# david-wb/tiny-diffusion

Measured on AMD Instinct MI355X. Metric: train images/s (q_sample+fwd+MSE+bwd+allreduce+Adam), MNIST 28x28 UNet fp32; 1000-step sample latency in `sample`, higher is better.
Workload: dtype f32; 1 GPU; diffusion.py unconditional MNIST 28x28 UNet, fp32, train step, batch 256/GPU (BASELINE.json configs[1]); global_batch=256, per_gpu_batch=256, parallelism=dp1

## Files before the change

include/tdx.h:

```cpp
#ifndef TDX_H
#define TDX_H

#include <stddef.h>
#include <stdint.h>

#ifdef __cplusplus
extern "C" {
#endif

#define TDX_VERSION 400

#define TDX_E_BADARG (-1)
#define TDX_E_SHAPE (-2)
#define TDX_E_WORKSPACE (-3)
#define TDX_E_STATE (-4)

typedef void* tdx_stream_t;

int tdx_version(void);
const char* tdx_error_string(int code);


int tdx_q_sample(const float* x0, const float* noise, const int64_t* t,
                 const float* sqrt_ac, const float* sqrt_1mac, float* x_t,
// ... 70 lines not shown
int tdx_initial_conv_input_grad(const float* g_out, const float* w, float* g_x, int B, int H, int W, int cin,
                                int cout, tdx_stream_t stream);
int tdx_final_conv_forward(const float* in, const float* w, const float* bias, float* out, int B, int H, int W,
                           int cout, tdx_stream_t stream);
int tdx_final_conv_backward(const float* in, const float* g_out, const float* w, float* g_in, float* dw, float* db,
                            float* scratch, int B, int H, int W, int cout, tdx_stream_t stream);

int tdx_conv3x3_fwd(const float* in, const float* wpk, const float* bias, float* out,
                    int B, int H, int W, int cin, int cout, int flags,
                    const float* in_scale, const float* in_shift,
                    const float* out_scale, const float* out_shift,
                    float* stats_partial, tdx_stream_t stream);
int tdx_conv3x3_fwd_splitk(const float* in, const float* wpk, const float* bias, float* out,
                           int B, int H, int W, int cin, int cout, int flags,
                           const float* in_scale, const float* in_shift,
                           const float* out_scale, const float* out_shift,
                           float* scratch, size_t scratch_floats, tdx_stream_t stream);
size_t tdx_conv3x3_splitk_scratch_floats(int B, int H, int W, int cin, int cout);
int tdx_conv3x3_wino_ok(int B, int H, int W, int cin, int cout);
int tdx_pack_conv3x3_wino(const float* w_oihw, float* u_fwd, float* u_dgrad, int cout, int cin, tdx_stream_t stream);
int tdx_conv3x3_fwd_wino(const float* in, const float* u, const float* bias, float* out, int B, int H, int W,
                         int cin, int cout, int flags, const float* out_scale, const float* out_shift,
                         float* stats_partial, tdx_stream_t stream);
int tdx_conv3x3_fwd_wino_infer(const float* in, const float* u, const float* bias, float* out, int B, int H, int W,
                               int cin, int cout, const float* out_scale, const float* out_shift, float* scratch,
                               size_t scratch_floats, tdx_stream_t stream);
int tdx_conv3x3_train_algo(int B, int H, int W, int cin, int cout, int role);
int tdx_conv3x3_infer_algo(int B, int H, int W, int cin, int cout);
int tdx_conv3x3_wgrad_wino_splits(int B, int H, int W, int cin, int cout);
int tdx_conv3x3_wgrad_wino(const float* in, const float* dy, float* dw_slabs, int B, int H, int W, int cin, int cout,
                           tdx_stream_t stream);
int tdx_conv3x3_wino_stat_tiles(int B, int H, int W);
int tdx_conv3x3_wino_stat_tile_rows(int B, int H, int W);
int tdx_pack_conv3x3_tiled(const float* w_oihw, float* w_tiled, int cout, int cin, tdx_stream_t stream);
int tdx_conv3x3_fwd_infer(const float* in, const float* w_tiled, const float* bias, float* out, int B, int H, int W,
                          int cin, int cout, const float* out_scale, const float* out_shift, float* scratch,
                          size_t scratch_floats, tdx_stream_t stream);
size_t tdx_conv3x3_infer_scratch_floats(int B, int H, int W, int cin, int cout);
int tdx_conv3x3_fwd_train(const float* in, const float* wpk, const float* bias, float* out, int B, int H, int W,
                          int cin, int cout, int flags, float* stats_partial, float* scratch,
                          size_t scratch_floats, tdx_stream_t stream);
size_t tdx_conv3x3_train_scratch_floats(int B, int H, int W, int cin, int cout);
int tdx_conv3x3_stat_tiles(int B, int H, int W, int cin, int cout);
int tdx_conv3x3_stat_tile_rows(int B, int H, int W, int cin, int cout);
int tdx_conv3x3_shape_ok(int B, int H, int W, int cin, int cout);
int tdx_conv3x3_tile_shape(int B, int H, int W, int cin, int cout, int role);
// ... 193 lines not shown
```

tiny_diffusion_amd/_lib.py:

```python
from __future__ import annotations

import ctypes as C
import os

import torch

from . import _build

_c_float_p = C.c_void_p
_c_i64_p = C.c_void_p
_ptr = C.c_void_p


class TdxError(RuntimeError):
    pass


def _load():
    path = _build.LIB
    if not os.path.exists(path):
        if os.environ.get("TDX_NO_AUTOBUILD"):
            raise TdxError(
                f"{path} not found: build it with `python -m tiny_diffusion_amd._build` "
                "(there is no CPU fallback for the HIP path)"
# ... 26 lines not shown
    "tdx_p_sample_step": (C.c_int, [_ptr, _ptr, _ptr, _ptr, _ptr, _ptr, C.c_int64, _ptr]),
    "tdx_p_sample_step_philox": (C.c_int, [_ptr, _ptr, _ptr, _ptr, _ptr, C.c_int64, C.c_uint64, _ptr]),
    "tdx_u8_gather_normalize": (C.c_int, [_ptr, _ptr, _ptr, C.c_int, C.c_int, C.c_float, C.c_float, _ptr]),
    "tdx_mse_loss": (C.c_int, [_ptr, _ptr, _ptr, _ptr, C.c_float, C.c_int64, _ptr]),
    "tdx_mse_scratch_bytes": (C.c_size_t, []),
    "tdx_mse_loss_grad": (C.c_int, [_ptr, _ptr, _ptr, _ptr, C.c_float, C.c_int64, _ptr, _ptr]),
    "tdx_adam_step": (C.c_int, [_ptr, _ptr, _ptr, _ptr, C.c_int64, C.c_float, C.c_float, C.c_float,
                                C.c_float, C.c_int, C.c_float, _ptr]),
    "tdx_adam_clip_scratch_bytes": (C.c_size_t, []),
    "tdx_adam_step_clip": (C.c_int, [_ptr, _ptr, _ptr, _ptr, C.c_int64, C.c_float, C.c_float, C.c_float, C.c_float,
                                     C.c_int, C.c_float, C.c_float, _ptr, _ptr, _ptr]),
    "tdx_edge_conv_wgrad_scratch_floats": (C.c_size_t, [C.c_int] * 3),
    "tdx_initial_conv_forward": (C.c_int, [_ptr, _ptr, _ptr, _ptr, C.c_int, C.c_int, C.c_int, C.c_int, C.c_int, _ptr]),
    "tdx_initial_conv_backward": (C.c_int, [_ptr, _ptr, _ptr, _ptr, _ptr, C.c_int, C.c_int, C.c_int, C.c_int, C.c_int,
                                            _ptr]),
    "tdx_final_conv_forward": (C.c_int, [_ptr, _ptr, _ptr, _ptr, C.c_int, C.c_int, C.c_int, C.c_int, _ptr]),
    "tdx_final_conv_backward": (C.c_int, [_ptr, _ptr, _ptr, _ptr, _ptr, _ptr, _ptr, C.c_int, C.c_int, C.c_int, C.c_int,
                                          _ptr]),
    "tdx_pack_conv3x3": (C.c_int, [_ptr, _ptr, _ptr, C.c_int, C.c_int, _ptr]),
    "tdx_conv3x3_wino_ok": (C.c_int, [C.c_int] * 5),
    "tdx_pack_conv3x3_wino": (C.c_int, [_ptr, _ptr, _ptr, C.c_int, C.c_int, _ptr]),
    "tdx_conv3x3_fwd_wino": (C.c_int, [_ptr, _ptr, _ptr, _ptr, C.c_int, C.c_int, C.c_int, C.c_int, C.c_int, C.c_int, _ptr,
                                       _ptr, _ptr, _ptr]),
    "tdx_conv3x3_fwd_wino_infer": (C.c_int, [_ptr, _ptr, _ptr, _ptr, C.c_int, C.c_int, C.c_int, C.c_int, C.c_int, _ptr, _ptr,
                                             _ptr, C.c_size_t, _ptr]),
    "tdx_conv3x3_train_algo": (C.c_int, [C.c_int] * 6),
    "tdx_conv3x3_infer_algo": (C.c_int, [C.c_int] * 5),
    "tdx_conv3x3_wgrad_wino_splits": (C.c_int, [C.c_int] * 5),
    "tdx_conv3x3_wgrad_wino": (C.c_int, [_ptr, _ptr, _ptr, C.c_int, C.c_int, C.c_int, C.c_int, C.c_int, _ptr]),
    "tdx_conv3x3_wino_stat_tiles": (C.c_int, [C.c_int] * 3),
    "tdx_conv3x3_wino_stat_tile_rows": (C.c_int, [C.c_int] * 3),
    "tdx_pack_conv3x3_tiled": (C.c_int, [_ptr, _ptr, C.c_int, C.c_int, _ptr]),
    "tdx_conv3x3_fwd_infer": (C.c_int, [_ptr, _ptr, _ptr, _ptr, C.c_int, C.c_int, C.c_int, C.c_int, C.c_int, _ptr, _ptr,
                                        _ptr, C.c_size_t, _ptr]),
    "tdx_conv3x3_infer_scratch_floats": (C.c_size_t, [C.c_int] * 5),
    "tdx_conv3x3_fwd": (C.c_int, [_ptr, _ptr, _ptr, _ptr, C.c_int, C.c_int, C.c_int, C.c_int, C.c_int,
                                  C.c_int, _ptr, _ptr, _ptr, _ptr, _ptr, _ptr]),
    "tdx_conv3x3_fwd_splitk": (C.c_int, [_ptr, _ptr, _ptr, _ptr, C.c_int, C.c_int, C.c_int, C.c_int, C.c_int,
                                         C.c_int, _ptr, _ptr, _ptr, _ptr, _ptr, C.c_size_t, _ptr]),
    "tdx_conv3x3_splitk_scratch_floats": (C.c_size_t, [C.c_int] * 5),
    "tdx_conv3x3_fwd_train": (C.c_int, [_ptr, _ptr, _ptr, _ptr, C.c_int, C.c_int, C.c_int, C.c_int, C.c_int, C.c_int,
                                        _ptr, _ptr, C.c_size_t, _ptr]),
    "tdx_conv3x3_train_scratch_floats": (C.c_size_t, [C.c_int] * 5),
    "tdx_conv3x3_stat_tiles": (C.c_int, [C.c_int] * 5),
    "tdx_conv3x3_stat_tile_rows": (C.c_int, [C.c_int] * 5),
    "tdx_conv3x3_wgrad_splits": (C.c_int, [C.c_int] * 5),
# ... 142 lines not shown
```

tiny_diffusion_amd/csrc/conv3x3.hip:

```cpp
#include "internal.h"
#include <cstring>

#define BK 32
#define BKP 36

#include "conv_shared.h"

template <int BM, int BN, int EPI>
__global__ void __launch_bounds__(256)
conv3x3_igemm_kernel(ConvArgs a) {
  constexpr int WGM = 2, WGN = 2;
  constexpr int WTM = BM / WGM, WTN = BN / WGN;
  constexpr int TM = WTM / 32, TN = WTN / 32;
  constexpr int AI = BM / 32, BI = BN / 32;
  static_assert(TM >= 1 && TN >= 1, "wave tile must hold a 32x32 MFMA tile");

  extern __shared__ __attribute__((aligned(16))) float smem[];
  float* As = smem;
  float* Bs = smem + 2 * BM * BKP;

  const int tid = threadIdx.x;
  const int lane = tid & 63, wave = tid >> 6;
  const int l31 = lane & 31, half = lane >> 5;
  const int wm = wave / WGN, wn = wave % WGN;
// ... 737 lines not shown
  if (!strcmp(key, "time_proj_early")) { g_tdx_time_proj_early = value != 0; return 0; }
  if (!strcmp(key, "time_stage_diag")) { g_tdx_time_stage = value == 6 ? 6 : 14; return 0; }
  if (!strcmp(key, "time_l1_impl")) { g_tdx_time_l1_impl = value; return 0; }
  if (!strcmp(key, "input_copy")) { g_tdx_input_copy = value; return 0; }
  if (!strcmp(key, "conv_dbg")) { g_conv_dbg = value; return 0; }
  if (!strcmp(key, "bf16_materialize")) { g_tdx_bf16_materialize = value ? 1 : 0; return 0; }
  if (!strcmp(key, "bf16_thin")) { g_tdx_bf16_thin = value < 0 ? 0 : value; return 0; }
  if (!strcmp(key, "bf16_ring")) { g_tdx_bf16_ring = value ? 1 : 0; return 0; }
  if (!strcmp(key, "bf16_wgrad9")) { g_tdx_wgrad9 = value ? 1 : 0; return 0; }
  if (!strcmp(key, "bf16_wgrad_swz")) { g_tdx_wgrad_bf16s = value ? 1 : 0; return 0; }
  if (!strcmp(key, "conv_stamp")) { g_conv_stamp = value; g_tdx_probe_stamp = value; return 0; }
  if (!strcmp(key, "wgrad_small")) { g_wgrad_small = value; return 0; }
  if (!strcmp(key, "wino")) { g_tdx_wino = value != 0; return 0; }
  if (!strcmp(key, "wino_infer")) { g_tdx_wino_infer = value != 0; return 0; }
  if (!strcmp(key, "wino_infer_min_units")) { g_tdx_wino_infer_min_units = value >= 0 ? value : 700; return 0; }
  if (!strcmp(key, "wino_infer_ovh")) { g_wino_infer_ovh = value >= 0 ? value : 2; return 0; }
  if (!strcmp(key, "wino_infer_red")) { g_wino_infer_red = value >= 0 ? value : 3; return 0; }
  if (!strcmp(key, "wino_wgrad")) { g_tdx_wino_wgrad = value != 0; return 0; }
  if (!strcmp(key, "wino_wgrad_min_tiles")) { g_tdx_wino_wgrad_min_tiles = value > 0 ? value : 1024; return 0; }
  if (!strcmp(key, "wino_wgrad_target")) { g_tdx_wino_wgrad_target = value > 0 ? value : 512; return 0; }
  if (!strcmp(key, "wino_min_wgs")) { g_tdx_wino_min_wgs = value > 0 ? value : 1; return 0; }
  if (!strcmp(key, "wino_rows")) { g_tdx_wino_rows = value != 0; return 0; }
  if (!strcmp(key, "wino_rows_min_stages")) { g_tdx_wino_rows_min_stages = value > 0 ? value : 16; return 0; }
  if (!strcmp(key, "infer_ring")) { g_tdx_infer_ring = value != 0; return 0; }
  if (!strcmp(key, "infer_stages")) { g_infer_stages = value == 3 ? 3 : 4; return 0; }
  if (!strcmp(key, "infer_splits")) { g_infer_splits = value > 0 ? value : 0; return 0; }
  if (!strcmp(key, "infer_ovh")) { g_infer_ovh = value >= 0 ? value : 4; return 0; }
  if (!strcmp(key, "infer_red")) { g_infer_red = value >= 0 ? value : 12; return 0; }
  if (!strcmp(key, "infer_cus")) { g_tdx_infer_cus = value > 0 && value <= 256 ? value : 256; return 0; }
  if (!strcmp(key, "wgrad9_wgs")) { g_wgrad9_wgs = value > 0 ? value : 0; return 0; }
  if (!strcmp(key, "wgrad_target")) { g_wgrad_target = value > 0 ? value : 2048; return 0; }
  if (!strcmp(key, "wgrad_target_big")) { g_wgrad_target_big = value > 0 ? value : 0; return 0; }
  return TDX_E_BADARG;
}

static TileCfg pick_tile(int64_t M, int cout) {
  const TileCfg cands[3] = {{128, 128}, {128, 64}, {64, 64}};
  if (g_force_tile >= 1 && g_force_tile <= 3 && cout % cands[g_force_tile - 1].bn == 0)
    return cands[g_force_tile - 1];
  for (int i = 0; i < 3; ++i) {
    if (cout % cands[i].bn) continue;
    if (i == 2) return cands[i];
    const int64_t tiles = ((M + cands[i].bm - 1) / cands[i].bm) * (cout / cands[i].bn);
    if (tiles < g_min_tiles) continue;
    const int64_t rounds = (tiles + 255) / 256;
    if ((double)(rounds * 256) <= 1.035 * (double)tiles) return cands[i];
// ... 1165 lines not shown
```

tiny_diffusion_amd/csrc/conv3x3_wino.hip:

```cpp
#include "internal.h"
#include "conv_shared.h"

extern unsigned* g_tdx_diag_buffer;
extern size_t g_tdx_diag_bytes;
extern int g_tdx_probe_stamp;

constexpr int WT = 64;
constexpr int WN = 64;
constexpr int WK = 8;
constexpr int A_ST = 16 * WT * WK;
constexpr int B_ST = 16 * WN * WK;
constexpr int STAGE = A_ST + B_ST;

struct WinoArgs {
  const float* in;
  const float* u;
  const float* bias;
  float* out;
  const float* out_scale;
  const float* out_shift;
  float* stats;
  int B, H, W, Cin, Cout, th, tw, NT, tilesN, M;
  float rcp_tpi, rcp_tw;
  int per;
  int compact;
  unsigned long long* stamps;
};

constexpr int OLD = 68;
constexpr int TAB_OFF = 2 * STAGE;
typedef unsigned u32x4 __attribute__((ext_vector_type(4)));

template <int EPI, int XH = -1>
__device__ __forceinline__ void wino_epilogue(const WinoArgs& a, float* out, const float* bias, f32x16 (&acc)[16], float* smem,
                                              int tblk, int n0, int wm, int wn, int l31, int half, int tid,
                                              const f32x4* xin = nullptr) {
#if defined(__HIP_DEVICE_COMPILE__)
  const unsigned* tab = reinterpret_cast<const unsigned*>(smem + TAB_OFF);
  const int cl = wn * 32 + l31, col = n0 + cl;
  const float bv = bias ? bias[col] : 0.f;
  float osc = 1.f, osh = 0.f;
  if (EPI == EPI_BNRELU) { osc = a.out_scale[col]; osh = a.out_shift[col]; }
  float csum = 0.f, cnt = 0.f;
  float* ot = smem;
  f32x4 pv[8];
#pragma unroll
  for (int r = 0; r < 16; ++r) {
    if (XH >= 0 && (r & 3) == 0) {
#pragma unroll
      for (int p = 0; p < 8; ++p) pv[p] = xin[(p * 4 + (r >> 2)) * 64];
    }
    auto M = [&](int p) { return XH >= 0 && (p >> 3) != XH ? pv[p & 7][r & 3] : acc[p][r]; };
    float s0[4], s1[4];
#pragma unroll
    for (int nu = 0; nu < 4; ++nu) {
      s0[nu] = M(0 + nu) + M(4 + nu) + M(8 + nu);
// ... 9 lines not shown
      const bool ok = (m >> q) & 1u;
      if (XH < 0) ot[(tl * 4 + q) * OLD + cl] = val;
      csum += ok ? val : 0.f;
      cnt += ok ? 1.f : 0.f;
      y[q] = ok ? val : 0.f;
    }
    acc[0][r] = y[0]; acc[1][r] = y[1]; acc[4][r] = y[2]; acc[5][r] = y[3];
    acc[2][r] = (m & 1u) ? 1.f : 0.f;
    acc[3][r] = (m & 2u) ? 1.f : 0.f;
    acc[6][r] = (m & 4u) ? 1.f : 0.f;
    acc[7][r] = (m & 8u) ? 1.f : 0.f;
  }
  if (XH >= 0) {
    __syncthreads();
#pragma unroll
    for (int r = 0; r < 16; ++r) {
      const int tl = wm * 32 + (r & 3) + 8 * (r >> 2) + 4 * half;
      ot[(tl * 4 + 0) * OLD + cl] = acc[0][r]; ot[(tl * 4 + 1) * OLD + cl] = acc[1][r];
      ot[(tl * 4 + 2) * OLD + cl] = acc[4][r]; ot[(tl * 4 + 3) * OLD + cl] = acc[5][r];
    }
  }
  __syncthreads();
  {
    const auto rsrc_out = __builtin_amdgcn_make_buffer_rsrc(out, 0, (int)((int64_t)a.M * a.Cout * 4), 0x00020000);
    const int c4 = (tid & 15) * 4, q = (tid >> 4) & 3;
    const unsigned qoff = (unsigned)((((q >> 1) * a.W + (q & 1)) * a.Cout + n0 + c4) * 4);
    const uint2* tab2 = reinterpret_cast<const uint2*>(tab);
    const float* src = ot + (tid >> 4) * OLD + c4;
#pragma unroll
    for (int i = 0; i < 16; ++i) {
      const uint2 e = tab2[4 * i + (tid >> 6)];
      const unsigned off = ((e.y >> q) & 1u) ? e.x + qoff : 0x80000000u;
      const f32x4 v = *reinterpret_cast<const f32x4*>(src + i * 16 * OLD);
      __builtin_amdgcn_raw_buffer_store_b128(__builtin_bit_cast(u32x4, v), rsrc_out, off, 0, 0);
    }
  }
  if (EPI == EPI_STATS) {
    float* red = smem + 256 * OLD;
    const float s = csum + __shfl_xor(csum, 32, 64);
    const float n = cnt + __shfl_xor(cnt, 32, 64);
    if (half == 0) { red[wm * 64 + cl] = s; red[128 + wm * 64 + cl] = n; }
    __syncthreads();
    if (tid < 64) {
      const float ts = red[tid] + red[64 + tid];
      const float tn = red[128 + tid] + red[192 + tid];
      red[256 + tid] = tn > 0.f ? ts / tn : 0.f;
      a.stats[((size_t)tblk * 2 + 0) * a.Cout + n0 + tid] = ts;
    }
    __syncthreads();
    const float mean = red[256 + cl];
    float q = 0.f;
#pragma unroll
    for (int r = 0; r < 16; ++r) {
      const float d0 = acc[0][r] - mean, d1 = acc[1][r] - mean, d2 = acc[4][r] - mean, d3 = acc[5][r] - mean;
      q = fmaf(d0 * acc[2][r], d0, q); q = fmaf(d1 * acc[3][r], d1, q);
// ... 17 lines not shown

__device__ __forceinline__ int div_rcp(int n, int d, float r, int* rem) {
  int q = (int)((float)n * r);
  int m = n - q * d;
  if (m < 0) { --q; m += d; }
  else if (m >= d) { ++q; m -= d; }
  *rem = m;
  return q;
}

template <int EPI, bool SPLITK, bool ROWS>
__global__ void __launch_bounds__(256)
conv3x3_wino_kernel(WinoArgs a) {
#if defined(__HIP_DEVICE_COMPILE__)
  static_assert(!ROWS || (!SPLITK && EPI != EPI_BNRELU), "the row split serves the training launches only");
  typedef __attribute__((address_space(3))) void* lds_ptr_t;
  extern __shared__ __attribute__((aligned(16))) float smem[];
  const unsigned long long t_entry = a.stamps ? __builtin_amdgcn_s_memrealtime() : 0ull;
  const int tid = threadIdx.x;
  const int lane = tid & 63;
  const int wave = __builtin_amdgcn_readfirstlane(tid >> 6);
  const int l31 = lane & 31, half = lane >> 5;
  const int wm = ROWS ? wave & 1 : wave >> 1, wn = ROWS ? wave >> 1 : wave & 1;
  const int xb = blockIdx.x / (8 * a.tilesN), xr = blockIdx.x % (8 * a.tilesN);
  const int tblk = a.compact ? (int)blockIdx.x / a.tilesN : xb * 8 + (xr & 7);
  const int nblk = a.compact ? (int)blockIdx.x - tblk * a.tilesN : xr >> 3;
  const int T0 = tblk * WT;
  if (T0 >= a.NT) return;
  const int n0 = nblk * WN;
  const int tpi = a.th * a.tw;

  if (tid < WT) {
    const int T = T0 + tid;
    const bool tv = T < a.NT;
    int rem, tx;
    const int b = div_rcp(T, tpi, a.rcp_tpi, &rem);
    const int ty = div_rcp(rem, a.tw, a.rcp_tw, &tx);
    const bool r1 = 2 * ty + 1 < a.H, c1 = 2 * tx + 1 < a.W;
    unsigned* tab = reinterpret_cast<unsigned*>(smem + TAB_OFF);
    tab[2 * tid] = tv ? (unsigned)(((b * a.H + 2 * ty) * a.W + 2 * tx) * a.Cout * 4) : 0u;
    tab[2 * tid + 1] = tv ? (1u | (c1 ? 2u : 0u) | (r1 ? 4u : 0u) | (r1 && c1 ? 8u : 0u)) : 0u;
  }

  const auto rsrc_in = __builtin_amdgcn_make_buffer_rsrc(const_cast<float*>(a.in), 0, (int)((int64_t)a.M * a.Cin * 4), 0x00020000);
  const auto rsrc_u = __builtin_amdgcn_make_buffer_rsrc(const_cast<float*>(a.u), 0, a.Cout * 16 * a.Cin * 4, 0x00020000);
  constexpr unsigned OOB = 0x80000000u;
  unsigned a_off[4][2];
#pragma unroll
  for (int g = 0; g < 2; ++g) {
// ... 222 lines not shown
          if (p < 12) { xop(2 * p); xop(2 * p + 1); }
          else piece(2 * (p - 12), cb, s + 2);
          __builtin_amdgcn_sched_barrier(0);
          acc[p] = __builtin_amdgcn_mfma_f32_32x32x2f32(v[p][2], bq[cur][2], acc[p], 0, 0, 0);
          if (p < 12) bq[(p + 2) % 5] = *reinterpret_cast<const f32x4*>(Bb + (p + 2) * 512);
          if (p == 12) { nbq[0] = *reinterpret_cast<const f32x4*>(Bn); nbq[1] = *reinterpret_cast<const f32x4*>(Bn + 512); }
          if (p == 13) {
#pragma unroll
            for (int c = 0; c < 4; ++c) d[12 + c] = *reinterpret_cast<const f32x4*>(An + (12 + c) * 512);
          }
          if (p == 14) { v[0] = sub4(t1[0], t1[2]); v[1] = add4(t1[1], t1[2]); }
          if (p == 15) piece(7, cb, s + 2);
          __builtin_amdgcn_sched_barrier(0);
          acc[p] = __builtin_amdgcn_mfma_f32_32x32x2f32(v[p][3], bq[cur][3], acc[p], 0, 0, 0);
          if (p >= 12 && p < 15) piece(2 * (p - 12) + 1, cb, s + 2);
          __builtin_amdgcn_sched_barrier(0);
        }
      };
      if (PEEL) stage(std::true_type{}, 0);
      for (int s = PEEL ? 1 : 0; s < ns; ++s) stage(std::false_type{}, s);
      asm volatile("s_waitcnt vmcnt(0) lgkmcnt(0)\n\ts_barrier" ::: "memory");
    }
    if (a.stamps) { t_loop = __builtin_amdgcn_s_memrealtime(); c_loop = __builtin_amdgcn_s_memtime() - c_loop; }
    if (SPLITK)
      wino_epilogue<EPI_PLAIN>(a, a.out + (size_t)blockIdx.y * (size_t)a.M * a.Cout, nullptr, acc, smem, tblk, n0, wm, wn, l31, half, tid);
    else
      wino_epilogue<EPI>(a, a.out, a.bias, acc, smem, tblk, n0, wm, wn, l31, half, tid);
  }
  if (a.stamps && tid == 0) {
    asm volatile("s_waitcnt vmcnt(0)" ::: "memory");
    unsigned long long* o = a.stamps + 8 * ((size_t)blockIdx.y * gridDim.x + blockIdx.x);
    o[0] = t_entry; o[1] = t_issued; o[2] = t_landed; o[3] = t_loop; o[4] = __builtin_amdgcn_s_memrealtime();
    o[5] = c_loop;
    o[6] = __builtin_amdgcn_s_getreg(4 | (0 << 6) | (31 << 11));
    o[7] = __builtin_amdgcn_s_getreg(20 | (0 << 6) | (3 << 11)) & 0xf;
  }
#endif
}

__global__ void __launch_bounds__(512) pack_wino_batch_kernel(TdxWinoPackBatch b) {
  int u = 0;
  while (u + 1 < b.count && (int)blockIdx.x >= b.start[u + 1]) ++u;
  const int cin = b.cin[u], cout = b.cout[u], cin_real = b.cin_real[u];
  const int blk = blockIdx.x - b.start[u];
  const int nkb = cin / 8;
  const int cb = blk / nkb, kb = blk - cb * nkb;
  const int cl = threadIdx.x >> 3, k8 = threadIdx.x & 7;
  const int co = cb * 64 + cl, ci = kb * 8 + k8;
  float g[9];
// ... 67 lines not shown
  TDX_CHECK_LAUNCH();
  return 0;
}

int tdx_pack_conv3x3_wino_pad(const float* w_oihw, float* u_fwd, float* u_dgrad, int cout, int cin_real, int cin,
                              tdx_stream_t stream) {
  if (!w_oihw || cout <= 0 || cin <= 0 || cin_real <= 0 || cin_real > cin) return TDX_E_BADARG;
  if (cin % 64 || cout % 64) return TDX_E_SHAPE;
  if (!u_fwd && !u_dgrad) return 0;
  TdxWinoPackBatch b{};
  b.count = 1;
  b.w[0] = w_oihw; b.uf[0] = u_fwd; b.ud[0] = u_dgrad; b.cout[0] = cout; b.cin[0] = cin; b.cin_real[0] = cin_real;
  return tdx_pack_conv3x3_wino_batch(&b, stream);
}

extern "C" int tdx_pack_conv3x3_wino(const float* w_oihw, float* u_fwd, float* u_dgrad, int cout, int cin,
                                     tdx_stream_t stream) {
  return tdx_pack_conv3x3_wino_pad(w_oihw, u_fwd, u_dgrad, cout, cin, cin, stream);
}

int g_tdx_wino_rows = 1;
int g_tdx_wino_rows_min_stages = 16;

int tdx_conv3x3_wino_launch(const float* in, const float* u, const float* bias, float* out, int B, int H, int W,
                            int cin, int cout, int flags, const float* out_scale, const float* out_shift,
                            float* stats_partial, int splits, int per, tdx_stream_t stream) {
  if (!in || !u || !out) return TDX_E_BADARG;
  if (!tdx_conv3x3_wino_ok(B, H, W, cin, cout)) return TDX_E_SHAPE;
  if (flags & ~(TDX_CONV_OUT_BNRELU | TDX_CONV_OUT_STATS)) return TDX_E_BADARG;
  if ((flags & TDX_CONV_OUT_BNRELU) && (!out_scale || !out_shift)) return TDX_E_BADARG;
  if ((flags & TDX_CONV_OUT_STATS) && (!stats_partial || (flags & TDX_CONV_OUT_BNRELU))) return TDX_E_BADARG;
  if (splits < 1 || (splits > 1 && (per < 1 || (int64_t)per * (splits - 1) >= cin / WK))) return TDX_E_BADARG;
  WinoArgs a{};
  a.in = in; a.u = u; a.bias = bias; a.out = out; a.out_scale = out_scale; a.out_shift = out_shift;
  a.stats = stats_partial;
  a.B = B; a.H = H; a.W = W; a.Cin = cin; a.Cout = cout;
  a.th = (H + 1) / 2; a.tw = (W + 1) / 2;
  a.NT = B * a.th * a.tw;
  a.rcp_tpi = 1.0f / (float)(a.th * a.tw); a.rcp_tw = 1.0f / (float)a.tw;
  a.tilesN = cout / WN;
  a.M = B * H * W;
  a.per = per;
  a.compact = cdiv(a.NT, WT) < 64;
  const dim3 grid(a.compact ? cdiv(a.NT, WT) * a.tilesN : (cdiv(a.NT, WT) + 7) / 8 * 8 * a.tilesN, splits);
  a.stamps = g_tdx_probe_stamp == 3 && g_tdx_diag_buffer && (size_t)grid.x * grid.y * 64 <= g_tdx_diag_bytes
                 ? reinterpret_cast<unsigned long long*>(g_tdx_diag_buffer) : nullptr;
  const size_t lds = (size_t)2 * STAGE * sizeof(float) + WT * 2 * sizeof(unsigned);
  hipStream_t st = to_stream(stream);
#define TDX_WINO_LAUNCH(EPI_, SPL_, ROWS_)                                                                       \
  do {                                                                                                           \
    auto kern = conv3x3_wino_kernel<EPI_, SPL_, ROWS_>;                                                          \
    static bool attr_set = false;                                                                                \
    if (!attr_set) {                                                                                             \
      hipError_t e = hipFuncSetAttribute(reinterpret_cast<const void*>(kern),                                    \
                                         hipFuncAttributeMaxDynamicSharedMemorySize, (int)lds);                  \
      if (e != hipSuccess) return (int)e;                                                                        \
      attr_set = true;                                                                                           \
    }                                                                                                            \
    kern<<<grid, 256, lds, st>>>(a);                                                                             \
  } while (0)
  const bool rows = g_tdx_wino_rows && cin / WK >= g_tdx_wino_rows_min_stages;
  if (splits > 1) TDX_WINO_LAUNCH(EPI_PLAIN, true, false);
  else if (flags & TDX_CONV_OUT_BNRELU) TDX_WINO_LAUNCH(EPI_BNRELU, false, false);
  else if (flags & TDX_CONV_OUT_STATS) {
    if (rows) TDX_WINO_LAUNCH(EPI_STATS, false, true);
    else TDX_WINO_LAUNCH(EPI_STATS, false, false);
  } else if (rows) TDX_WINO_LAUNCH(EPI_PLAIN, false, true);
  else TDX_WINO_LAUNCH(EPI_PLAIN, false, false);
#undef TDX_WINO_LAUNCH
  TDX_CHECK_LAUNCH();
  return 0;
}

extern "C" int tdx_conv3x3_fwd_wino(const float* in, const float* u, const float* bias, float* out, int B, int H, int W,
                                    int cin, int cout, int flags, const float* out_scale, const float* out_shift,
                                    float* stats_partial, tdx_stream_t stream) {
  return tdx_conv3x3_wino_launch(in, u, bias, out, B, H, W, cin, cout, flags, out_scale, out_shift, stats_partial, 1, 0,
                                 stream);
}

constexpr int GT8 = 8;
constexpr int XS_F = GT8 * 16 * 64;
constexpr int ES_F = GT8 * 4 * 64;
constexpr int WST_F = XS_F + ES_F;
constexpr int WNST = 3;
constexpr int WG_MAX_CHUNK = 1024;
constexpr int WG_XCH_F = 4 * 8 * 16 * 64;
constexpr size_t WG_LDS = 131072;
static_assert((size_t)WNST * WST_F * 4 + (size_t)WG_MAX_CHUNK * 4 <= WG_LDS && (size_t)WG_XCH_F * 4 <= WG_LDS, "LDS");

struct WinoWgArgs {
  const float* in;
  const float* dy;
  float* slabs;
  int B, H, W, Cin, Cout, th, tw, NT, M;
  int tilesCo, tilesCi, chunk;
  unsigned long long* stamps;
};

#if defined(__HIP_DEVICE_COMPILE__)
__device__ __forceinline__ unsigned long long wg_lanes16(unsigned m) {
// ... 321 lines not shown
```

tiny_diffusion_amd/csrc/internal.h:

```cpp
#pragma once
#include "common.h"

int tdx_copy_floats(const float* src, float* dst, size_t n, hipStream_t st);
int tdx_copy_segments(const float* const* src, float* const* dst, const size_t* n, int count, hipStream_t st);
int tdx_pixel_sum(const void* g, float* out, int B, int HW, int C, hipStream_t st, int io16 = 0);
int tdx_reduce_partials(const float* partial, float* out, int nblk, int stride, int count,
                        hipStream_t st);
int tdx_initial_conv_fwd(const float* x, const float* w, const float* bias, void* out, int B, int H,
                         int W, int cin, int cout_real, hipStream_t st, int io16 = 0);
int tdx_small_conv_wgrad_blocks(int B, int H, int W);
int tdx_small_conv_partial_width(void);
int tdx_initial_conv_wgrad(const float* x, const void* g, float* partial, float* dw, float* db,
                           int B, int H, int W, int cin, int cout_real, hipStream_t st, int io16 = 0);
int tdx_initial_conv_dgrad(const void* g_x0, const float* w, float* g_x, int B, int H, int W, int cin,
                           int cout_real, hipStream_t st, int io16 = 0);
int tdx_final_conv_fwd(const void* in, const float* w, const float* bias, float* out, int B, int H,
                       int W, int cout, hipStream_t st, int io16 = 0);
int tdx_final_conv_fwd_psample(const void* in, const float* w, const float* bias, float* eps_out, int B, int H, int W,
                               int cout, float* x, const float* z, const float* coef, const int32_t* t_idx,
                               uint64_t seed, int philox, int64_t* counter_dec, hipStream_t st, int io16 = 0,
                               int64_t elem0 = 0, const int64_t* tau = nullptr, int guided = 0, float gw = 0.f);
int tdx_final_conv_dgrad(const float* g_out, const float* w, void* g_in, int B, int H, int W,
                         int cout, hipStream_t st, int io16 = 0);
int tdx_final_conv_wgrad(const void* in, const float* g_out, float* partial, float* dw, float* db,
// ... 23 lines not shown
#define TDX_PACK_MAX 13
struct TdxPackBatch {
  const float* w[TDX_PACK_MAX];
  float* wf[TDX_PACK_MAX];
  float* wd[TDX_PACK_MAX];
  int cout[TDX_PACK_MAX], cin[TDX_PACK_MAX], cin_real[TDX_PACK_MAX], chunk_start[TDX_PACK_MAX];
  int count;
};
int tdx_pack_conv3x3_batch(TdxPackBatch* b, tdx_stream_t stream);
struct TdxWinoPackBatch {
  const float* w[TDX_PACK_MAX];
  float* uf[TDX_PACK_MAX];
  float* ud[TDX_PACK_MAX];
  int cout[TDX_PACK_MAX], cin[TDX_PACK_MAX], cin_real[TDX_PACK_MAX], start[TDX_PACK_MAX];
  int count;
};
int tdx_pack_conv3x3_wino_batch(TdxWinoPackBatch* b, tdx_stream_t stream);
extern "C" int tdx_conv3x3_wino_ok(int B, int H, int W, int cin, int cout);
extern "C" int tdx_conv3x3_wino_stat_tiles(int B, int H, int W);
extern "C" int tdx_conv3x3_wino_stat_tile_rows(int B, int H, int W);
extern int g_tdx_wino, g_tdx_wino_min_wgs;
extern int g_tdx_wino_wgrad, g_tdx_wino_wgrad_min_tiles, g_tdx_wino_wgrad_target;
extern int g_tdx_wino_rows, g_tdx_wino_rows_min_stages;
extern "C" int tdx_conv3x3_wgrad_wino_splits(int B, int H, int W, int cin, int cout);
extern "C" int tdx_conv3x3_wgrad_wino(const float* in, const float* dy, float* dw_slabs, int B, int H, int W, int cin, int cout,
                                      tdx_stream_t stream);
extern int g_tdx_wino_infer_min_units;
extern int g_tdx_wino_infer;
int tdx_conv3x3_wino_launch(const float* in, const float* u, const float* bias, float* out, int B, int H, int W,
                            int cin, int cout, int flags, const float* out_scale, const float* out_shift,
                            float* stats_partial, int splits, int per, tdx_stream_t stream);
int tdx_conv3x3_fwd_wino_infer_ex(const float* in, const float* u, const float* bias, float* out, int B, int H, int W,
                                  int cin, int cout, const float* out_scale, const float* out_shift, float* scratch,
                                  size_t scratch_floats, tdx_stream_t stream, TdxSplitDefer* defer, TdxPoolFuse* pool);
int tdx_pack_conv3x3_tiled_batch(TdxPackBatch* b, tdx_stream_t stream);
int tdx_pack_conv3x3_tiled_pad(const float* w_oihw, float* w_tiled, int cout, int cin_real, int cin, tdx_stream_t stream);
int tdx_pack_conv3x3_batch_bf16(TdxPackBatch* b, tdx_stream_t stream);
int tdx_pack_conv3x3_pad(const float* w_oihw, float* w_fwd, float* w_dgrad, int cout, int cin_real,
                         int cin, tdx_stream_t stream);
int tdx_conv3x3_wgrad_reduce_pad(const float* dw_slabs, float* dw_oihw, int splits, int cout, int cin,
                                 int cin_real, tdx_stream_t stream);
int tdx_time_embed_bwd_ex(const float* tf, const int64_t* y, const float* const* P, float* const* G,
                          const float* pre, const float* emb, const float* const* gk, const int* ldg,
                          const int* widths, float* scratch, int B, int ncls, hipStream_t st,
                          const int64_t* t_i64 = nullptr, int td = 0, int parts = 7);
int tdx_bn_moments(const float* stats_partial, int tiles, int tile_rows, int64_t count, int C, double* mom,
// ... 77 lines not shown
```

tiny_diffusion_amd/csrc/unet.hip:

```cpp
#include "internal.h"
#include <algorithm>
#include <cstdlib>
#include <mutex>
#include <new>
#include <string>
#include <vector>

namespace {

struct UnitDef {
  int cin, cout, hw;
  int in_bn;
  int cin_real;
};

struct NetSpec {
  int in_ch, hw0, out_hw;
  int x0_ch, x0_real;
  int overlap;
  int time_dim;
  int enc_hw[4];
  int dec_hw[3];
  int skip_ch[3];
  UnitDef units[13];
// ... 50 lines not shown
Layout make_layout(const NetSpec& S, int B) {
  Layout L;
  size_t o = 0;
  auto take = [&](size_t n) { size_t r = o; o += align64(n); return r; };
  const size_t b = (size_t)B;
  const size_t px0 = (size_t)S.hw0 * S.hw0;
  L.x = take(b * px0 * S.in_ch); L.t = take(2 * b); L.y = take(std::max<size_t>(2 * b, b * S.time_dim));
  L.sin = take(b * S.time_dim); L.pre = take(b * S.time_dim); L.emb = take(b * S.time_dim);
  for (int k = 0; k < 3; ++k) L.tp[k] = take(b * S.skip_ch[k]);
  L.x0 = take(b * px0 * S.x0_ch);
  size_t stats = 0, slabs = 0, bnscr = 0, gbuf = 0, ksplit = 0;
  for (int u = 0; u < 13; ++u) {
    const UnitDef& d = S.units[u];
    L.Y[u] = take(b * d.hw * d.hw * d.cout);
    L.ss[u] = take(4 * (size_t)d.cout);
    L.A[u] = (u + 1 < 13 && S.units[u + 1].in_bn) ? take(b * d.hw * d.hw * d.cout) : 0;
    stats = std::max(stats, (size_t)tdx_conv3x3_stat_tiles(B, d.hw, d.hw, d.cin, d.cout) * 2 * d.cout);
    slabs = std::max(slabs, (size_t)std::max(std::max(tdx_conv3x3_wgrad_splits(B, d.hw, d.hw, d.cin, d.cout),
                                                      tdx_conv3x3_wgrad_splits_bf16(B, d.hw, d.hw, d.cin, d.cout)),
                                             tdx_conv3x3_wgrad_wino_splits(B, d.hw, d.hw, d.cin, d.cout)) *
                                9 * (size_t)d.cin * d.cout);
    ksplit = std::max(ksplit, std::max(tdx_conv3x3_train_scratch_floats(B, d.hw, d.hw, d.cin, d.cout),
                                       tdx_conv3x3_train_scratch_floats(B, d.hw, d.hw, d.cout, d.cin)));
    bnscr = std::max(bnscr, tdx_bn_relu_bwd_scratch_floats((int64_t)b * d.hw * d.hw, d.cout));
    gbuf = std::max(gbuf, b * d.hw * d.hw * (size_t)std::max(d.cin, d.cout));
  }
  for (int k = 0; k < 3; ++k) {
    const int hp = S.enc_hw[k + 1];
    L.ep[k] = take(b * hp * hp * S.skip_ch[k]);
  }
  for (int k = 0; k < 3; ++k) {
    const UnitDef& d = S.units[7 + 2 * k];
    L.cat[k] = take(b * d.hw * d.hw * d.cin);
  }
  L.d1a = take(b * S.out_hw * S.out_hw * 64);
  gbuf = std::max(gbuf, b * (size_t)S.out_hw * S.out_hw * 64);
  L.stats = take(stats);
  L.ksplit_floats = ksplit;
  L.ksplit = take(ksplit);
  L.gbuf = gbuf;
  L.G1 = take(gbuf); L.G2 = take(gbuf); L.G3 = take(gbuf); L.G4 = take(gbuf);
  for (int k = 0; k < 3; ++k) {
    L.GS[k] = take(b * S.enc_hw[k] * S.enc_hw[k] * S.skip_ch[k]);
    L.gtp[k] = take(b * S.skip_ch[k]);
  }
  L.slabs = take(slabs);
// ... 586 lines not shown
                                 on_load ? sh(i - 1) : nullptr, nullptr, nullptr, ws + L.stats, io16, stream));
      const int rows = tdx_conv3x3_bf16_stat_tile_rows();
      RC(finalize_bn(i, cdiv(M, rows), rows, M));
      if (mat16 && i + 1 < 13 && S.units[i + 1].in_bn)
        RC(tdx_bn_relu_apply(Y, ws + L.A[i], M, d.cout, ss, ss + d.cout, st, 1));
      return 0;
    }
    if (infer) {
      const float* iss = u->infer_ss + u->iss_off[i];
      if (u->wino_f[i] && tdx_conv3x3_infer_algo(B, d.hw, d.hw, d.cin, d.cout))
        return tdx_conv3x3_fwd_wino_infer_ex(in, u->upack + u->uf_off[i], bias, Y, B, d.hw, d.hw, d.cin, d.cout, iss,
                                             iss + d.cout, ws + L.G1, 2 * L.gbuf, stream, defer, pool);
      if (u->wf_tiled)
        return tdx_conv3x3_fwd_infer_ex(in, wf, bias, Y, B, d.hw, d.hw, d.cin, d.cout, iss, iss + d.cout, ws + L.G1,
                                        2 * L.gbuf, stream, defer, pool);
      return tdx_conv3x3_fwd_splitk_fused(in, wf, bias, Y, B, d.hw, d.hw, d.cin, d.cout, TDX_CONV_OUT_BNRELU, iss,
                                          iss + d.cout, ws + L.G1, 2 * L.gbuf, u->kcount, TDX_KCOUNT, stream, defer,
                                          pool);
    }
    const bool bn_on_load = d.in_bn && !u->materialize;
    if (d.in_bn && u->materialize) in = ws + L.A[i - 1];
    int flags = (bn_on_load ? TDX_CONV_IN_BNRELU : 0) | (training ? TDX_CONV_OUT_STATS : 0);
    if (u->wino_f[i] && !bn_on_load) {
      RC(tdx_conv3x3_fwd_wino(in, u->upack + u->uf_off[i], bias, Y, B, d.hw, d.hw, d.cin, d.cout,
                              training ? TDX_CONV_OUT_STATS : 0, nullptr, nullptr, ws + L.stats, stream));
      RC(finalize_bn(i, tdx_conv3x3_wino_stat_tiles(B, d.hw, d.hw), tdx_conv3x3_wino_stat_tile_rows(B, d.hw, d.hw),
                     (int64_t)B * d.hw * d.hw));
      if (u->materialize && i + 1 < 13 && S.units[i + 1].in_bn)
        RC(tdx_bn_relu_apply(Y, ws + L.A[i], (int64_t)B * d.hw * d.hw, d.cout, ss, ss + d.cout, st));
      return 0;
    }
    if (bn_on_load)
      RC(tdx_conv3x3_fwd(in, wf, bias, Y, B, d.hw, d.hw, d.cin, d.cout, flags, sc(i - 1), sh(i - 1), nullptr, nullptr,
                         ws + L.stats, stream));
    else
      RC(tdx_conv3x3_fwd_train(in, wf, bias, Y, B, d.hw, d.hw, d.cin, d.cout, flags, ws + L.stats, ws + L.ksplit,
                               L.ksplit_floats, stream));
    const int tiles = tdx_conv3x3_stat_tiles(B, d.hw, d.hw, d.cin, d.cout);
    RC(finalize_bn(i, tiles, tdx_conv3x3_stat_tile_rows(B, d.hw, d.hw, d.cin, d.cout), (int64_t)B * d.hw * d.hw));
    if (u->materialize && i + 1 < 13 && S.units[i + 1].in_bn)
      RC(tdx_bn_relu_apply(Y, ws + L.A[i], (int64_t)B * d.hw * d.hw, d.cout, ss, ss + d.cout, st));
    return 0;
  };

  RC(run_unit(0, ws + L.x0));
  if (!infer) RC(pack_tail(u, params, stream));
  for (int k = 0; k < 3; ++k) {
    const int ua = 2 * k, ub = 2 * k + 1;
// ... 546 lines not shown
```

Baseline: 27040 images/s.

## Split-K the Winograd forward tail wave to fill idle CUs

Adds a tail-balancing path to the Winograd forward conv used in training. The workgroups that fall into the last partial wave (wgs mod slot count) are relaunched with K split into S slices. Each slice writes dense partials to scratch, and a reduce kernel sums them, adds bias, scatters to the output and computes the per-tile BN sum and M2 stats. Full waves still run the normal fused kernel. The aim is to cut tail-wave underutilisation, at the cost of extra launches, scratch traffic and a separate reduction pass.

```diff
diff --git a/include/tdx.h b/include/tdx.h
--- a/include/tdx.h
+++ b/include/tdx.h
@@ -116,6 +116,11 @@
 int tdx_conv3x3_fwd_wino(const float* in, const float* u, const float* bias, float* out, int B, int H, int W,
                          int cin, int cout, int flags, const float* out_scale, const float* out_shift,
                          float* stats_partial, tdx_stream_t stream);
+int tdx_conv3x3_wino_tail_plan(int B, int H, int W, int cin, int cout, int* full_blocks, int* tail_blocks, int* slices);
+size_t tdx_conv3x3_wino_tail_scratch_floats(int B, int H, int W, int cin, int cout);
+int tdx_conv3x3_wino_launch_tail(const float* in, const float* u, const float* bias, float* out, int B, int H, int W,
+                                 int cin, int cout, float* stats_partial, float* scratch, size_t scratch_floats,
+                                 tdx_stream_t stream);
 int tdx_conv3x3_fwd_wino_infer(const float* in, const float* u, const float* bias, float* out, int B, int H, int W,
                                int cin, int cout, const float* out_scale, const float* out_shift, float* scratch,
                                size_t scratch_floats, tdx_stream_t stream);
diff --git a/tiny_diffusion_amd/_lib.py b/tiny_diffusion_amd/_lib.py
--- a/tiny_diffusion_amd/_lib.py
+++ b/tiny_diffusion_amd/_lib.py
@@ -72,6 +72,9 @@
     "tdx_pack_conv3x3_wino": (C.c_int, [_ptr, _ptr, _ptr, C.c_int, C.c_int, _ptr]),
     "tdx_conv3x3_fwd_wino": (C.c_int, [_ptr, _ptr, _ptr, _ptr, C.c_int, C.c_int, C.c_int, C.c_int, C.c_int, C.c_int, _ptr,
                                        _ptr, _ptr, _ptr]),
+    "tdx_conv3x3_wino_tail_plan": (C.c_int, [C.c_int] * 5 + [_ptr] * 3),
+    "tdx_conv3x3_wino_tail_scratch_floats": (C.c_size_t, [C.c_int] * 5),
+    "tdx_conv3x3_wino_launch_tail": (C.c_int, [_ptr] * 4 + [C.c_int] * 5 + [_ptr, _ptr, C.c_size_t, _ptr]),
     "tdx_conv3x3_fwd_wino_infer": (C.c_int, [_ptr, _ptr, _ptr, _ptr, C.c_int, C.c_int, C.c_int, C.c_int, C.c_int, _ptr, _ptr,
                                              _ptr, C.c_size_t, _ptr]),
     "tdx_conv3x3_train_algo": (C.c_int, [C.c_int] * 6),
diff --git a/tiny_diffusion_amd/csrc/conv3x3.hip b/tiny_diffusion_amd/csrc/conv3x3.hip
--- a/tiny_diffusion_amd/csrc/conv3x3.hip
+++ b/tiny_diffusion_amd/csrc/conv3x3.hip
@@ -783,6 +783,9 @@
   if (!strcmp(key, "wino_min_wgs")) { g_tdx_wino_min_wgs = value > 0 ? value : 1; return 0; }
   if (!strcmp(key, "wino_rows")) { g_tdx_wino_rows = value != 0; return 0; }
   if (!strcmp(key, "wino_rows_min_stages")) { g_tdx_wino_rows_min_stages = value > 0 ? value : 16; return 0; }
+  if (!strcmp(key, "wino_tail")) { g_tdx_wino_tail = value != 0; return 0; }
+  if (!strcmp(key, "wino_tail_slots")) { g_tdx_wino_tail_slots = value > 0 ? value : 256; return 0; }
+  if (!strcmp(key, "wino_tail_min_stages")) { g_tdx_wino_tail_min_stages = value > 0 ? value : 8; return 0; }
   if (!strcmp(key, "infer_ring")) { g_tdx_infer_ring = value != 0; return 0; }
   if (!strcmp(key, "infer_stages")) { g_infer_stages = value == 3 ? 3 : 4; return 0; }
   if (!strcmp(key, "infer_splits")) { g_infer_splits = value > 0 ? value : 0; return 0; }
diff --git a/tiny_diffusion_amd/csrc/conv3x3_wino.hip b/tiny_diffusion_amd/csrc/conv3x3_wino.hip
--- a/tiny_diffusion_amd/csrc/conv3x3_wino.hip
+++ b/tiny_diffusion_amd/csrc/conv3x3_wino.hip
@@ -25,13 +25,24 @@
   int per;
   int compact;
   unsigned long long* stamps;
+  int bid0, unit0, tail_units, ntb;
+  float* part;
 };
+
+__host__ __device__ inline int wino_unit_to_bid(int u, int tilesN, int ntb, int compact, int* tblk, int* nblk) {
+  if (compact) { *tblk = u / tilesN; *nblk = u - *tblk * tilesN; return u; }
+  const int g = 8 * tilesN, xb = u / g, j = u - xb * g;
+  const int v = ntb - 8 * xb < 8 ? ntb - 8 * xb : 8;
+  *nblk = j / v;
+  *tblk = xb * 8 + (j - *nblk * v);
+  return xb * g + *nblk * 8 + (j - *nblk * v);
+}
 
 constexpr int OLD = 68;
 constexpr int TAB_OFF = 2 * STAGE;
 typedef unsigned u32x4 __attribute__((ext_vector_type(4)));
 
-template <int EPI, int XH = -1>
+template <int EPI, int XH = -1, bool DENSE = false>
 __device__ __forceinline__ void wino_epilogue(const WinoArgs& a, float* out, const float* bias, f32x16 (&acc)[16], float* smem,
                                               int tblk, int n0, int wm, int wn, int l31, int half, int tid,
                                               const f32x4* xin = nullptr) {
@@ -87,7 +98,8 @@
   }
   __syncthreads();
   {
-    const auto rsrc_out = __builtin_amdgcn_make_buffer_rsrc(out, 0, (int)((int64_t)a.M * a.Cout * 4), 0x00020000);
+    const bool dense = DENSE && a.part != nullptr;
+    const auto rsrc_out = __builtin_amdgcn_make_buffer_rsrc(out, 0, dense ? 256 * WN * 4 : (int)((int64_t)a.M * a.Cout * 4), 0x00020000);
     const int c4 = (tid & 15) * 4, q = (tid >> 4) & 3;
     const unsigned qoff = (unsigned)((((q >> 1) * a.W + (q & 1)) * a.Cout + n0 + c4) * 4);
     const uint2* tab2 = reinterpret_cast<const uint2*>(tab);
@@ -95,7 +107,7 @@
 #pragma unroll
     for (int i = 0; i < 16; ++i) {
       const uint2 e = tab2[4 * i + (tid >> 6)];
-      const unsigned off = ((e.y >> q) & 1u) ? e.x + qoff : 0x80000000u;
+      const unsigned off = dense ? (unsigned)(((i * 16 + (tid >> 4)) * WN + c4) * 4) : ((e.y >> q) & 1u) ? e.x + qoff : 0x80000000u;
       const f32x4 v = *reinterpret_cast<const f32x4*>(src + i * 16 * OLD);
       __builtin_amdgcn_raw_buffer_store_b128(__builtin_bit_cast(u32x4, v), rsrc_out, off, 0, 0);
     }
@@ -159,9 +171,10 @@
   const int wave = __builtin_amdgcn_readfirstlane(tid >> 6);
   const int l31 = lane & 31, half = lane >> 5;
   const int wm = ROWS ? wave & 1 : wave >> 1, wn = ROWS ? wave >> 1 : wave & 1;
-  const int xb = blockIdx.x / (8 * a.tilesN), xr = blockIdx.x % (8 * a.tilesN);
-  const int tblk = a.compact ? (int)blockIdx.x / a.tilesN : xb * 8 + (xr & 7);
-  const int nblk = a.compact ? (int)blockIdx.x - tblk * a.tilesN : xr >> 3;
+  const int bid = (int)blockIdx.x + a.bid0;
+  const int xb = bid / (8 * a.tilesN), xr = bid % (8 * a.tilesN);
+  const int tblk = a.compact ? bid / a.tilesN : xb * 8 + (xr & 7);
+  const int nblk = a.compact ? bid - tblk * a.tilesN : xr >> 3;
   const int T0 = tblk * WT;
   if (T0 >= a.NT) return;
   const int n0 = nblk * WN;
@@ -430,9 +443,15 @@
       asm volatile("s_waitcnt vmcnt(0) lgkmcnt(0)\n\ts_barrier" ::: "memory");
     }
     if (a.stamps) { t_loop = __builtin_amdgcn_s_memrealtime(); c_loop = __builtin_amdgcn_s_memtime() - c_loop; }
-    if (SPLITK)
-      wino_epilogue<EPI_PLAIN>(a, a.out + (size_t)blockIdx.y * (size_t)a.M * a.Cout, nullptr, acc, smem, tblk, n0, wm, wn, l31, half, tid);
-    else
+    if (SPLITK) {
+      float* dst = a.out + (size_t)blockIdx.y * (size_t)a.M * a.Cout;
+      if (a.part) {
+        const int v = min(8, a.ntb - 8 * xb);
+        const int unit = a.compact ? bid : xb * 8 * a.tilesN + (xr >> 3) * v + (xr & 7);
+        dst = a.part + ((size_t)blockIdx.y * a.tail_units + (unit - a.unit0)) * (size_t)(256 * WN);
+      }
+      wino_epilogue<EPI_PLAIN, -1, true>(a, dst, nullptr, acc, smem, tblk, n0, wm, wn, l31, half, tid);
+    } else
       wino_epilogue<EPI>(a, a.out, a.bias, acc, smem, tblk, n0, wm, wn, l31, half, tid);
   }
   if (a.stamps && tid == 0) {
@@ -546,9 +565,14 @@
 int g_tdx_wino_rows = 1;
 int g_tdx_wino_rows_min_stages = 16;
 
-int tdx_conv3x3_wino_launch(const float* in, const float* u, const float* bias, float* out, int B, int H, int W,
+struct WinoSub {
+  int bid0, nbid;
+  float* part;
+  int unit0, tail_units;
+};
+static int wino_launch_impl(const float* in, const float* u, const float* bias, float* out, int B, int H, int W,
                             int cin, int cout, int flags, const float* out_scale, const float* out_shift,
-                            float* stats_partial, int splits, int per, tdx_stream_t stream) {
+                            float* stats_partial, int splits, int per, tdx_stream_t stream, const WinoSub* sub) {
   if (!in || !u || !out) return TDX_E_BADARG;
   if (!tdx_conv3x3_wino_ok(B, H, W, cin, cout)) return TDX_E_SHAPE;
   if (flags & ~(TDX_CONV_OUT_BNRELU | TDX_CONV_OUT_STATS)) return TDX_E_BADARG;
@@ -565,8 +589,14 @@
   a.tilesN = cout / WN;
   a.M = B * H * W;
   a.per = per;
-  a.compact = cdiv(a.NT, WT) < 64;
-  const dim3 grid(a.compact ? cdiv(a.NT, WT) * a.tilesN : (cdiv(a.NT, WT) + 7) / 8 * 8 * a.tilesN, splits);
+  a.ntb = cdiv(a.NT, WT);
+  a.compact = a.ntb < 64;
+  dim3 grid(a.compact ? a.ntb * a.tilesN : (a.ntb + 7) / 8 * 8 * a.tilesN, splits);
+  if (sub) {
+    if (sub->bid0 < 0 || sub->nbid < 1 || sub->bid0 + sub->nbid > (int)grid.x) return TDX_E_BADARG;
+    a.bid0 = sub->bid0; a.part = sub->part; a.unit0 = sub->unit0; a.tail_units = sub->tail_units;
+    grid.x = sub->nbid;
+  }
   a.stamps = g_tdx_probe_stamp == 3 && g_tdx_diag_buffer && (size_t)grid.x * grid.y * 64 <= g_tdx_diag_bytes
                  ? reinterpret_cast<unsigned long long*>(g_tdx_diag_buffer) : nullptr;
   const size_t lds = (size_t)2 * STAGE * sizeof(float) + WT * 2 * sizeof(unsigned);
@@ -596,11 +626,157 @@
   return 0;
 }
 
+int tdx_conv3x3_wino_launch(const float* in, const float* u, const float* bias, float* out, int B, int H, int W,
+                            int cin, int cout, int flags, const float* out_scale, const float* out_shift,
+                            float* stats_partial, int splits, int per, tdx_stream_t stream) {
+  return wino_launch_impl(in, u, bias, out, B, H, W, cin, cout, flags, out_scale, out_shift, stats_partial, splits, per,
+                          stream, nullptr);
+}
+
 extern "C" int tdx_conv3x3_fwd_wino(const float* in, const float* u, const float* bias, float* out, int B, int H, int W,
                                     int cin, int cout, int flags, const float* out_scale, const float* out_shift,
                                     float* stats_partial, tdx_stream_t stream) {
   return tdx_conv3x3_wino_launch(in, u, bias, out, B, H, W, cin, cout, flags, out_scale, out_shift, stats_partial, 1, 0,
                                  stream);
+}
+
+int g_tdx_wino_tail = 1;
+int g_tdx_wino_tail_slots = 256;
+int g_tdx_wino_tail_min_stages = 8;
+
+static int wino_tail_plan(int B, int H, int W, int cin, int cout, bool enabled, int* full_blocks, int* tail_blocks,
+                          int* slices) {
+  if (!tdx_conv3x3_wino_ok(B, H, W, cin, cout)) return TDX_E_SHAPE;
+  const int wgs = tdx_conv3x3_wino_stat_tiles(B, H, W) * (cout / WN);
+  const int slots = g_tdx_wino_tail_slots, stages = cin / WK;
+  const int R = wgs % slots;
+  int S = 1;
+  if (enabled && R > 0)
+    for (int s = std::min(slots / R, stages / g_tdx_wino_tail_min_stages); s >= 2; --s)
+      if (stages % s == 0) { S = s; break; }
+  if (full_blocks) *full_blocks = S > 1 ? wgs - R : wgs;
+  if (tail_blocks) *tail_blocks = S > 1 ? R : 0;
+  if (slices) *slices = S;
+  return 0;
+}
+
+extern "C" int tdx_conv3x3_wino_tail_plan(int B, int H, int W, int cin, int cout, int* full_blocks, int* tail_blocks,
+                                          int* slices) {
+  return wino_tail_plan(B, H, W, cin, cout, g_tdx_wino_tail != 0, full_blocks, tail_blocks, slices);
+}
+
+extern "C" size_t tdx_conv3x3_wino_tail_scratch_floats(int B, int H, int W, int cin, int cout) {
+  int full, tail, S;
+  if (wino_tail_plan(B, H, W, cin, cout, true, &full, &tail, &S)) return 0;
+  return (size_t)tail * S * 256 * WN;
+}
+
+struct WinoTailArgs {
+  const float* part;
+  const float* bias;
+  float* out;
+  float* stats;
+  int H, W, Cout, th, tw, NT, tilesN, ntb, compact, unit0, S;
+  size_t slab;
+};
+
+__global__ void __launch_bounds__(1024) wino_tail_reduce_kernel(WinoTailArgs a) {
+  __shared__ unsigned tab[2 * WT];
+  __shared__ float red[64 * WN], redn[64], mean[WN];
+  const int tid = threadIdx.x, pr = tid >> 4, c4 = (tid & 15) * 4;
+  int tblk, nblk;
+  wino_unit_to_bid(a.unit0 + (int)blockIdx.x, a.tilesN, a.ntb, a.compact, &tblk, &nblk);
+  const int n0 = nblk * WN;
+  if (tid < WT) {
+    const int T = tblk * WT + tid, tpi = a.th * a.tw;
+    const bool tv = T < a.NT;
+    const int b = T / tpi, rem = T - b * tpi, ty = rem / a.tw, tx = rem - ty * a.tw;
+    const bool r1 = 2 * ty + 1 < a.H, c1 = 2 * tx + 1 < a.W;
+    tab[2 * tid] = tv ? (unsigned)(((b * a.H + 2 * ty) * a.W + 2 * tx) * a.Cout) : 0u;
+    tab[2 * tid + 1] = tv ? (1u | (c1 ? 2u : 0u) | (r1 ? 4u : 0u) | (r1 && c1 ? 8u : 0u)) : 0u;
+  }
+  __syncthreads();
+  const float* src = a.part + (size_t)blockIdx.x * (256 * WN) + pr * WN + c4;
+  f32x4 v[4];
+#pragma unroll
+  for (int i = 0; i < 4; ++i) v[i] = *reinterpret_cast<const f32x4*>(src + i * 64 * WN);
+  for (int s = 1; s < a.S; ++s) {
+#pragma unroll
+    for (int i = 0; i < 4; ++i) v[i] += *reinterpret_cast<const f32x4*>(src + (size_t)s * a.slab + i * 64 * WN);
+  }
+  f32x4 bv = {0.f, 0.f, 0.f, 0.f};
+  if (a.bias) bv = *reinterpret_cast<const f32x4*>(a.bias + n0 + c4);
+  f32x4 csum = {0.f, 0.f, 0.f, 0.f};
+  float okf[4], cnt = 0.f;
+  const int q = pr & 3;
+#pragma unroll
+  for (int i = 0; i < 4; ++i) {
+    const int tl = 16 * i + (pr >> 2);
+    const bool ok = (tab[2 * tl + 1] >> q) & 1u;
+    v[i] += bv;
+    if (ok) *reinterpret_cast<f32x4*>(a.out + (size_t)tab[2 * tl] + ((q >> 1) * a.W + (q & 1)) * a.Cout + n0 + c4) = v[i];
+    okf[i] = ok ? 1.f : 0.f;
+    cnt += okf[i];
+    if (ok) csum += v[i];
+  }
+#pragma unroll
+  for (int k = 0; k < 4; ++k) red[pr * WN + c4 + k] = csum[k];
+  if ((tid & 15) == 0) redn[pr] = cnt;
+  __syncthreads();
+  if (tid < WN) {
+    float ts = 0.f, tn = 0.f;
+    for (int r = 0; r < 64; ++r) { ts += red[r * WN + tid]; tn += redn[r]; }
+    mean[tid] = tn > 0.f ? ts / tn : 0.f;
+    a.stats[((size_t)tblk * 2 + 0) * a.Cout + n0 + tid] = ts;
+  }
+  __syncthreads();
+  f32x4 m2 = {0.f, 0.f, 0.f, 0.f};
+#pragma unroll
+  for (int i = 0; i < 4; ++i)
+#pragma unroll
+    for (int k = 0; k < 4; ++k) {
+      const float d = v[i][k] - mean[c4 + k];
+      m2[k] = fmaf(d * okf[i], d, m2[k]);
+    }
+#pragma unroll
+  for (int k = 0; k < 4; ++k) red[pr * WN + c4 + k] = m2[k];
+  __syncthreads();
+  if (tid < WN) {
+    float t = 0.f;
+    for (int r = 0; r < 64; ++r) t += red[r * WN + tid];
+    a.stats[((size_t)tblk * 2 + 1) * a.Cout + n0 + tid] = t;
+  }
+}
+
+extern "C" int tdx_conv3x3_wino_launch_tail(const float* in, const float* u, const float* bias, float* out, int B, int H,
+                                            int W, int cin, int cout, float* stats_partial, float* scratch,
+                                            size_t scratch_floats, tdx_stream_t stream) {
+  if (!in || !u || !out || !stats_partial) return TDX_E_BADARG;
+  int full, tail, S;
+  if (int rc = tdx_conv3x3_wino_tail_plan(B, H, W, cin, cout, &full, &tail, &S)) return rc;
+  if (S == 1)
+    return tdx_conv3x3_wino_launch(in, u, bias, out, B, H, W, cin, cout, TDX_CONV_OUT_STATS, nullptr, nullptr,
+                                   stats_partial, 1, 0, stream);
+  if (!scratch || scratch_floats < (size_t)tail * S * 256 * WN) return TDX_E_BADARG;
+  WinoTailArgs t{};
+  t.part = scratch; t.bias = bias; t.out = out; t.stats = stats_partial;
+  t.H = H; t.W = W; t.Cout = cout; t.th = (H + 1) / 2; t.tw = (W + 1) / 2;
+  t.NT = B * t.th * t.tw; t.tilesN = cout / WN; t.ntb = cdiv(t.NT, WT); t.compact = t.ntb < 64;
+  t.unit0 = full; t.S = S; t.slab = (size_t)tail * 256 * WN;
+  const int gridx = t.compact ? t.ntb * t.tilesN : (t.ntb + 7) / 8 * 8 * t.tilesN;
+  int tb, nb;
+  const int bid0 = wino_unit_to_bid(full, t.tilesN, t.ntb, t.compact, &tb, &nb);
+  const WinoSub st{bid0, gridx - bid0, scratch, full, tail};
+  if (int rc = wino_launch_impl(in, u, nullptr, out, B, H, W, cin, cout, 0, nullptr, nullptr, nullptr, S, cin / WK / S,
+                                stream, &st)) return rc;
+  if (full > 0) {
+    const WinoSub sf{0, bid0, nullptr, 0, 0};
+    if (int rc = wino_launch_impl(in, u, bias, out, B, H, W, cin, cout, TDX_CONV_OUT_STATS, nullptr, nullptr,
+                                  stats_partial, 1, 0, stream, &sf)) return rc;
+  }
+  wino_tail_reduce_kernel<<<tail, 1024, 0, to_stream(stream)>>>(t);
+  TDX_CHECK_LAUNCH();
+  return 0;
 }
 
 constexpr int GT8 = 8;
diff --git a/tiny_diffusion_amd/csrc/internal.h b/tiny_diffusion_amd/csrc/internal.h
--- a/tiny_diffusion_amd/csrc/internal.h
+++ b/tiny_diffusion_amd/csrc/internal.h
@@ -69,6 +69,13 @@
 extern int g_tdx_wino, g_tdx_wino_min_wgs;
 extern int g_tdx_wino_wgrad, g_tdx_wino_wgrad_min_tiles, g_tdx_wino_wgrad_target;
 extern int g_tdx_wino_rows, g_tdx_wino_rows_min_stages;
+extern int g_tdx_wino_tail, g_tdx_wino_tail_slots, g_tdx_wino_tail_min_stages;
+extern "C" int tdx_conv3x3_wino_tail_plan(int B, int H, int W, int cin, int cout, int* full_blocks, int* tail_blocks,
+                                          int* slices);
+extern "C" size_t tdx_conv3x3_wino_tail_scratch_floats(int B, int H, int W, int cin, int cout);
+extern "C" int tdx_conv3x3_wino_launch_tail(const float* in, const float* u, const float* bias, float* out, int B, int H,
+                                            int W, int cin, int cout, float* stats_partial, float* scratch,
+                                            size_t scratch_floats, tdx_stream_t stream);
 extern "C" int tdx_conv3x3_wgrad_wino_splits(int B, int H, int W, int cin, int cout);
 extern "C" int tdx_conv3x3_wgrad_wino(const float* in, const float* dy, float* dw_slabs, int B, int H, int W, int cin, int cout,
                                       tdx_stream_t stream);
diff --git a/tiny_diffusion_amd/csrc/unet.hip b/tiny_diffusion_amd/csrc/unet.hip
--- a/tiny_diffusion_amd/csrc/unet.hip
+++ b/tiny_diffusion_amd/csrc/unet.hip
@@ -96,6 +96,7 @@
                                 9 * (size_t)d.cin * d.cout);
     ksplit = std::max(ksplit, std::max(tdx_conv3x3_train_scratch_floats(B, d.hw, d.hw, d.cin, d.cout),
                                        tdx_conv3x3_train_scratch_floats(B, d.hw, d.hw, d.cout, d.cin)));
+    ksplit = std::max(ksplit, tdx_conv3x3_wino_tail_scratch_floats(B, d.hw, d.hw, d.cin, d.cout));
     bnscr = std::max(bnscr, tdx_bn_relu_bwd_scratch_floats((int64_t)b * d.hw * d.hw, d.cout));
     gbuf = std::max(gbuf, b * d.hw * d.hw * (size_t)std::max(d.cin, d.cout));
   }
@@ -728,8 +729,12 @@
     if (d.in_bn && u->materialize) in = ws + L.A[i - 1];
     int flags = (bn_on_load ? TDX_CONV_IN_BNRELU : 0) | (training ? TDX_CONV_OUT_STATS : 0);
     if (u->wino_f[i] && !bn_on_load) {
-      RC(tdx_conv3x3_fwd_wino(in, u->upack + u->uf_off[i], bias, Y, B, d.hw, d.hw, d.cin, d.cout,
-                              training ? TDX_CONV_OUT_STATS : 0, nullptr, nullptr, ws + L.stats, stream));
+      if (training)
+        RC(tdx_conv3x3_wino_launch_tail(in, u->upack + u->uf_off[i], bias, Y, B, d.hw, d.hw, d.cin, d.cout, ws + L.stats,
+                                        ws + L.ksplit, L.ksplit_floats, stream));
+      else
+        RC(tdx_conv3x3_fwd_wino(in, u->upack + u->uf_off[i], bias, Y, B, d.hw, d.hw, d.cin, d.cout, 0, nullptr, nullptr,
+                                ws + L.stats, stream));
       RC(finalize_bn(i, tdx_conv3x3_wino_stat_tiles(B, d.hw, d.hw), tdx_conv3x3_wino_stat_tile_rows(B, d.hw, d.hw),
                      (int64_t)B * d.hw * d.hw));
       if (u->materialize && i + 1 < 13 && S.units[i + 1].in_bn)
```

Result: no change. 27230 images/s, median of 6 (+0.7%).
